# nnaisense/evotorch

Hardware: NVIDIA H100
Metric: PGPE generations/sec at popsize=1Mxdim=10k (Rastrigin, fp32) (higher is better)
Workload: dtype f32

## Files before the change

evotorch_b200/_native.py:

```python

from __future__ import annotations

import ctypes
import os
from ctypes import c_float, c_int, c_int64, c_size_t, c_uint64, c_void_p
from typing import Optional

import torch

_PKG = os.path.dirname(os.path.abspath(__file__))
LIB_PATH = os.path.join(_PKG, "lib", "libevok.so")

_P = c_void_p
_SIGNATURES = {
    "evok_abi_version": (c_int, []),
    "evok_launch_count": (c_uint64, []),
    "evok_error_string": (ctypes.c_char_p, [c_int]),
    "evok_sample_eval": (c_int, [c_int, _P, c_int64, _P, _P, c_int64, c_int64, c_int64, c_int, c_uint64, c_uint64, _P, _P, _P]),
    "evok_eval": (c_int, [c_int, _P, c_int64, c_int64, c_int64, _P, _P]),
    "evok_objective_register": (c_int, [_P, c_size_t, _P, c_int, _P]),
    "evok_objective_load": (c_int, [c_int]),
    "evok_rank_workspace_bytes": (c_size_t, [c_int64]),
    "evok_rank": (c_int, [c_int, _P, c_int64, c_int, _P, _P, _P, c_size_t, _P]),
    "evok_argsort": (c_int, [_P, c_int64, c_int, _P, _P, c_size_t, _P]),
    "evok_sample_batched": (c_int, [_P, c_int64, c_int64, _P, c_int64, _P, c_int64, c_int64, c_int64, c_int64, c_int, c_uint64, c_uint64, _P]),
    "evok_rank_batched": (c_int, [c_int, _P, c_int64, c_int64, c_int, _P, _P, c_size_t, _P]),
    "evok_elite_mask_batched": (c_int, [_P, c_int64, c_int64, c_int64, _P, _P, c_size_t, _P]),
    "evok_weights_adjust_batched": (c_int, [_P, c_int64, c_int64, c_int, _P]),
    "evok_grad_batched_workspace_bytes": (c_size_t, [c_int64, c_int64, c_int64]),
    "evok_grad_batched": (c_int, [c_int, _P, c_int64, c_int64, _P, _P, c_int64, _P, c_int64, c_int64, c_int64, c_int64, c_float, c_float, _P, _P, _P,
                                  c_size_t, _P]),
    "evok_clipup_batched": (c_int, [_P, c_int64, c_int64, _P, _P, _P, _P, _P, _P]),
    "evok_sigma_update_batched": (c_int, [_P, _P, c_int64, c_int64, _P, c_int, _P, _P, _P, _P]),
    "evok_rank_table": (c_int, [_P, c_int64, c_int, _P, _P, _P, c_size_t, _P]),
    "evok_cholesky_workspace_bytes": (c_size_t, [c_int64]),
    "evok_cholesky": (c_int, [_P, c_int64, c_int64, _P, c_int64, _P, c_size_t, _P]),
    "evok_cmaes_row_weights": (c_int, [_P, _P, c_int64, c_int64, c_int64, c_int, _P, _P, _P]),
    "evok_cmaes_vector_update": (c_int, [_P, _P, c_int64, _P, _P, _P, _P, _P, c_int64, _P, c_int, _P, _P, _P]),
    "evok_sample_eval_sq": (c_int, [c_int, _P, c_int64, _P, _P, c_int64, c_int64, c_int64, c_uint64, c_uint64, _P, _P, _P, _P]),
    "evok_sepcma_workspace_bytes": (c_size_t, [c_int64, c_int64]),
    "evok_sepcma_moments": (c_int, [_P, _P, c_int, c_int64, c_int64, c_int64, c_uint64, c_uint64, _P, _P, _P, _P, _P, c_size_t, _P]),
    "evok_sepcma_update": (c_int, [_P, _P, _P, c_int64, _P, _P, _P, _P, _P, _P, _P, _P, _P, _P, c_int64, _P, c_int, c_int64, c_float, c_float, _P,
                                   _P]),
    "evok_weights_adjust": (c_int, [_P, c_int64, c_int, _P]),
    "evok_elite_mask": (c_int, [_P, c_int64, c_int64, _P, _P, c_size_t, _P]),
    "evok_grad_workspace_bytes": (c_size_t, [c_int64, c_int64]),
    "evok_grad": (c_int, [c_int, _P, c_int64, _P, _P, _P, c_int64, c_int64, c_float, c_float, _P, _P, _P, c_size_t, _P]),
    "evok_grad_regen": (c_int, [c_int, _P, _P, _P, c_int64, c_int64, c_int64, c_uint64, c_uint64, _P, c_float, c_float, _P, _P, _P,
                                c_size_t, _P]),
    "evok_grad_hybrid": (c_int, [c_int, _P, c_int64, _P, _P, _P, c_int64, c_int64, c_int64, c_uint64, c_uint64, _P, c_int, c_float, c_float, _P,
                                 _P, _P, c_size_t, _P]),
    "evok_grad_auto_split": (c_int, [c_int64]),
    "evok_grad_power_limit_mw": (c_int64, [c_int]),
    "evok_clipup_step": (c_int, [_P, c_int64, _P, c_float, c_float, c_float, _P, _P, _P]),
    "evok_adam_step": (c_int, [_P, c_int64, _P, _P, c_int64, c_float, c_float, c_float, c_float, _P, _P, _P]),
    "evok_sgd_step": (c_int, [_P, c_int64, _P, c_int, c_float, c_float, _P, _P, _P]),
    "evok_axpy": (c_int, [_P, c_int64, c_float, _P, _P]),
    "evok_sigma_update": (c_int, [_P, _P, c_int64, c_float, c_int, _P, c_float, _P, c_float, _P, c_float, _P]),
    "evok_cem_finalize": (c_int, [_P, _P, _P, c_int64, c_int64, _P, _P, _P]),
    "evok_mlp_parameter_length": (c_int64, [c_int, _P]),
    "evok_mlp_forward": (c_int, [_P, c_int64, _P, c_int64, _P, c_int64, c_int64, c_int, _P, _P, _P]),
    "evok_mlp_forward_prep": (c_int, [_P, c_int64, _P, c_int64, _P, c_int64, c_int64, c_int, _P, _P, _P, _P, _P, c_float, c_float, c_float, _P, _P,
                                      c_size_t, _P]),
    "evok_mlp_forward_shared_supported": (c_int, [c_int, _P]),
    "evok_mlp_forward_shared_workspace_bytes": (c_size_t, [c_int64, c_int64, c_int, _P]),
    "evok_mlp_forward_shared": (c_int, [_P, c_int64, c_int64, _P, c_int64, c_int64, c_int, _P, _P, _P, _P, c_size_t, _P]),
    "evok_gemm_gather_rows": (c_int, [_P, c_int64, c_int64, c_int64, c_int64, _P, c_int64, c_int64, c_int64, c_int64, c_int, _P, c_int64, _P]),
    "evok_gemm_gather_rows_workspace_bytes": (c_size_t, [c_int64, c_int64]),
    "evok_gemm_gather_rows_ws": (c_int, [_P, c_int64, c_int64, c_int64, c_int64, _P, c_int64, c_int64, c_int64, c_int64, c_int, _P, c_int64, c_int, _P, c_size_t, _P]),
    "evok_gemm_workspace_bytes": (c_size_t, [c_int64, c_int64, c_int64]),
    "evok_gemm_nt": (c_int, [_P, c_int64, _P, c_int64, c_int64, c_int64, c_int64, _P, c_int64, _P, c_int64, _P, _P, _P, c_size_t, _P]),
    "evok_gemm_nt_affine": (c_int, [_P, c_int64, _P, c_int64, c_int64, c_int64, c_int64, _P, c_int64, _P, _P, c_int64, _P, _P, c_size_t, _P]),
    "evok_transpose_pair": (c_int, [_P, c_int64, c_int64, c_int64, _P, _P, _P, c_int64, _P]),
    "evok_transpose_scale": (c_int, [_P, c_int64, c_int64, c_int64, _P, _P, c_int64, _P]),
    "evok_peer_alloc": (c_int, [c_size_t, _P, _P]),
    "evok_peer_open": (c_int, [_P, _P]),
    "evok_peer_close": (c_int, [_P]),
    "evok_peer_free": (c_int, [_P]),
    "evok_sample_eval_push": (c_int, [c_int, _P, c_int64, _P, _P, c_int64, c_int64, c_int64, c_int, c_uint64, c_uint64, _P, c_int, c_int, _P, _P,
                                      _P, _P, _P]),
    "evok_peer_push": (c_int, [_P, c_int64, c_int64, c_int, c_int, _P, _P, _P, _P]),
    "evok_peer_wait": (c_int, [_P, c_int, _P, _P, c_uint64, _P]),
    "evok_grad_push": (c_int, [c_int, _P, c_int64, _P, _P, _P, c_int64, c_int64, c_int64, c_uint64, c_uint64, _P, c_float, c_float, c_int, c_int,
                               _P, _P, _P, _P, _P, c_size_t, _P]),
    "evok_rank_sharded": (c_int, [c_int, _P, c_int64, c_int, c_int, c_int, _P, _P, _P, _P, _P, _P, _P, c_uint64, _P, _P, _P, c_size_t, _P]),
    "evok_peer_reduce": (c_int, [_P, c_int, c_int64, _P, _P, _P, _P, c_uint64, _P, _P]),
}

EXPORTED_SYMBOLS = tuple(sorted(_SIGNATURES))

_lib: Optional[ctypes.CDLL] = None


class EvokError(RuntimeError):
    pass


def lib() -> ctypes.CDLL:
    global _lib
    if _lib is None:
        if not os.path.exists(LIB_PATH):
            raise EvokError(
                f"{LIB_PATH} is missing: the sm_90a kernel library has not been built. "
                "Run `python -m evotorch_b200.build` (needs nvcc). There is no CPU/torch fallback for CUDA problems."
# ... 72 lines not shown
```

evotorch_b200/csrc/evok_grad.cu:

```cuda
#include <dlfcn.h>

#include <atomic>
#include <cstdlib>

#include "evok_common.cuh"

#ifndef EVOK_GRAD_TMA_DEFAULT
#define EVOK_GRAD_TMA_DEFAULT 1
#endif

namespace evok {

#ifndef EVOK_GRAD_UNROLL
#define EVOK_GRAD_UNROLL 4
#endif
#ifndef EVOK_GRAD_MINB
#define EVOK_GRAD_MINB 4
#endif
#ifndef EVOK_GRAD_CTAS_PER_SM
#define EVOK_GRAD_CTAS_PER_SM 4
#endif
constexpr int kGradThreads = 256;
constexpr int kGradUnroll = EVOK_GRAD_UNROLL;
constexpr int kMaxResidentCtas = kNumSMs * 8;
// ... 199 lines not shown
  }
  out_mu[j] = t1 * scale_mu;
  out_sigma[j] = t2 * scale_sigma;
}

struct GradPush {
  PeerSink sink;
  const unsigned long long* epoch;
  unsigned int* done;
};

__global__ void __launch_bounds__(256) grad_finalize_push_kernel(const float* __restrict__ partial, int n_chunks, int64_t D, float scale_mu,
                                                                 float scale_sigma, const __grid_constant__ PeerSink sink,
                                                                 const unsigned long long* epoch, unsigned int* done) {
  const int64_t j = (int64_t)blockIdx.x * blockDim.x + threadIdx.x;
  if (j < D) {
    float t1 = 0.0f, t2 = 0.0f;
    for (int c = 0; c < n_chunks; ++c) {
      t1 += partial[((int64_t)c * 2 + 0) * D + j];
      t2 += partial[((int64_t)c * 2 + 1) * D + j];
    }
    t1 *= scale_mu;
    t2 *= scale_sigma;
    for (int p = 0; p < sink.world; ++p) {
      float* slot = static_cast<float*>(sink.data[p]) + (int64_t)sink.rank * 2 * D;
      slot[j] = t1;
      slot[D + j] = t2;
    }
  }
  peer_signal_tail(sink, epoch, done);
}

static int launch_finalize(const float* partial, int n_chunks, int64_t D, float scale_mu, float scale_sigma, float* out_mu, float* out_sigma,
                           const GradPush* push, cudaStream_t st) {
  const unsigned grid = (unsigned)((D + 255) / 256);
  if (push) grad_finalize_push_kernel<<<grid, 256, 0, st>>>(partial, n_chunks, D, scale_mu, scale_sigma, push->sink, push->epoch, push->done);
  else grad_finalize_kernel<<<grid, 256, 0, st>>>(partial, n_chunks, D, scale_mu, scale_sigma, out_mu, out_sigma);
  EVOK_CHECK_LAUNCH();
  return 0;
}

#ifndef EVOK_GRAD_TMA_ROWS
#define EVOK_GRAD_TMA_ROWS 4
#endif
#ifndef EVOK_GRAD_TMA_STAGES
#define EVOK_GRAD_TMA_STAGES 4
#endif
#ifndef EVOK_GRAD_TMA_CTAS_PER_SM
#define EVOK_GRAD_TMA_CTAS_PER_SM 3
#endif
constexpr int kTmaRows = EVOK_GRAD_TMA_ROWS;
constexpr int kTmaStages = EVOK_GRAD_TMA_STAGES;
constexpr int kTmaCols = 1024;
constexpr int kTmaConsumers = 256;
constexpr int kTmaThreads = kTmaConsumers + 32;
constexpr size_t kTmaSmemBytes = (size_t)kTmaStages * kTmaRows * kTmaCols * sizeof(float) + 2 * kTmaStages * sizeof(uint64_t) + 128;

__device__ __forceinline__ uint32_t smem_u32(const void* p) { return (uint32_t)__cvta_generic_to_shared(p); }
__device__ __forceinline__ void mbar_init(uint64_t* bar, uint32_t count) {
  asm volatile("mbarrier.init.shared::cta.b64 [%0], %1;" ::"r"(smem_u32(bar)), "r"(count) : "memory");
}
__device__ __forceinline__ void mbar_expect_tx(uint64_t* bar, uint32_t bytes) {
  asm volatile("mbarrier.arrive.expect_tx.shared::cta.b64 _, [%0], %1;" ::"r"(smem_u32(bar)), "r"(bytes) : "memory");
}
__device__ __forceinline__ void mbar_arrive(uint64_t* bar) {
  asm volatile("mbarrier.arrive.shared::cta.b64 _, [%0];" ::"r"(smem_u32(bar)) : "memory");
}
__device__ __forceinline__ void mbar_wait(uint64_t* bar, uint32_t parity) {
  asm volatile(
      "{\n"
      ".reg .pred P1;\n"
      "LAB_WAIT:\n"
      "mbarrier.try_wait.parity.shared::cta.b64 P1, [%0], %1;\n"
      "@P1 bra DONE;\n"
      "bra LAB_WAIT;\n"
      "DONE:\n"
      "}" ::"r"(smem_u32(bar)), "r"(parity) : "memory");
}
__device__ __forceinline__ void bulk_load(void* dst_smem, const void* src_gmem, uint32_t bytes, uint64_t* bar) {
  asm volatile("cp.async.bulk.shared::cluster.global.mbarrier::complete_tx::bytes [%0], [%1], %2, [%3];" ::"r"(smem_u32(dst_smem)),
               "l"(src_gmem), "r"(bytes), "r"(smem_u32(bar))
               : "memory");
}

constexpr int kSplitPeriod = 16;
__device__ __forceinline__ uint32_t rebuilt_mask(int split) {
  uint32_t m = 0;
#pragma unroll
  for (int k = 0; k < kSplitPeriod; ++k)
    if ((k + 1) * split / kSplitPeriod > k * split / kSplitPeriod) m |= 1u << k;
  return m;
}
__device__ __forceinline__ bool group_rebuilt(uint32_t mask, int64_t g) { return (mask >> ((int)g & (kSplitPeriod - 1))) & 1u; }

template <bool SYM>
__global__ void __launch_bounds__(kTmaThreads, EVOK_GRAD_TMA_CTAS_PER_SM)
    grad_partial_tma_kernel(int form, const float* __restrict__ X, int64_t ldx, const float* __restrict__ w, const float* __restrict__ mu,
                            const float* __restrict__ sigma, int64_t n_units, int64_t D, int64_t units_per_chunk, int split, uint64_t unit0,
                            const __grid_constant__ PhiloxKey key, const uint32_t* __restrict__ stream_off, float* __restrict__ partial) {
  extern __shared__ __align__(128) unsigned char smem_raw[];
  float* tiles = reinterpret_cast<float*>(smem_raw);
  uint64_t* full = reinterpret_cast<uint64_t*>(smem_raw + (size_t)kTmaStages * kTmaRows * kTmaCols * sizeof(float));
  uint64_t* empty = full + kTmaStages;

  const int tid = threadIdx.x, warp = tid >> 5, lane = tid & 31;
  const int64_t col0 = (int64_t)blockIdx.x * kTmaCols;
  const int64_t width = min((int64_t)kTmaCols, D - col0);
  const int64_t r_begin = (int64_t)blockIdx.y * units_per_chunk;
  const int64_t r_end = min(n_units, r_begin + units_per_chunk);
  const int64_t n_rows = r_end - r_begin;
  const int64_t n_groups = (n_rows + kTmaRows - 1) / kTmaRows;
  const int64_t row_stride = (SYM ? 2 : 1) * ldx;
  const uint32_t mask = rebuilt_mask(split);

  if (tid == 0) {
    for (int s = 0; s < kTmaStages; ++s) {
      mbar_init(&full[s], 1);
      mbar_init(&empty[s], kTmaConsumers / 32);
    }
    asm volatile("fence.mbarrier_init.release.cluster;" ::: "memory");
  }
  __syncthreads();

  if (warp == kTmaConsumers / 32) {
    if (lane == 0) {
      const uint32_t row_bytes = (uint32_t)(width * sizeof(float));
      int64_t t = 0;
      for (int64_t g = 0; g < n_groups; ++g) {
        if (group_rebuilt(mask, g)) continue;
        const int s = (int)(t % kTmaStages);
        const uint32_t use = (uint32_t)(t / kTmaStages);
        ++t;
        if (use > 0) mbar_wait(&empty[s], (use - 1) & 1);
        const int64_t r0 = r_begin + g * kTmaRows;
        const int rows = (int)min((int64_t)kTmaRows, r_end - r0);
        mbar_expect_tx(&full[s], rows * row_bytes);
        float* dst = tiles + (size_t)s * kTmaRows * kTmaCols;
        for (int i = 0; i < rows; ++i) bulk_load(dst + (size_t)i * kTmaCols, X + (r0 + i) * row_stride + col0, row_bytes, &full[s]);
      }
    }
    return;
  }

  const int64_t col = col0 + (int64_t)tid * 4;
  const bool active = col < D;
  const uint32_t sw = key.stream_lo + (stream_off ? __ldg(stream_off) : 0u);
  const int frm = SYM ? EVOK_GRAD_SYMMETRIC : form;
  float m[4], sg[4], c1[4], c0[4];
#pragma unroll
  for (int c = 0; c < 4; ++c) {
    sg[c] = active ? __ldg(sigma + col + c) : 1.0f;
    m[c] = active ? __ldg(mu + col + c) : 0.0f;
    if (frm == EVOK_GRAD_EXP) {
      c1[c] = __fdiv_rn(1.0f, sg[c] * sg[c]);
      c0[c] = 1.0f;
    } else if (frm == EVOK_GRAD_MOMENTS) {
      c1[c] = 1.0f;
      c0[c] = 0.0f;
    } else {
      c1[c] = __fdiv_rn(1.0f, sg[c]);
      c0[c] = sg[c];
    }
  }
  float s1[4] = {0.f, 0.f, 0.f, 0.f}, s2[4] = {0.f, 0.f, 0.f, 0.f};

  int64_t t = 0;
  for (int64_t g = 0; g < n_groups; ++g) {
    const int64_t r0 = r_begin + g * kTmaRows;
    const int rows = (int)min((int64_t)kTmaRows, r_end - r0);
    float a[kTmaRows], b[kTmaRows];
    bool need[kTmaRows];
#pragma unroll
    for (int i = 0; i < kTmaRows; ++i) {
      a[i] = b[i] = 0.0f;
      if (i < rows) {
        if (SYM) {
          const float wp = __ldg(w + 2 * (r0 + i)), wm = __ldg(w + 2 * (r0 + i) + 1);
          a[i] = 0.5f * (wp - wm);
          b[i] = 0.5f * (wp + wm);
        } else {
          a[i] = b[i] = __ldg(w + r0 + i);
        }
      }
      need[i] = a[i] != 0.0f || b[i] != 0.0f;
    }
    if (group_rebuilt(mask, g)) {
      if (active) {
        float x[kTmaRows][4];
#pragma unroll
        for (int i = 0; i < kTmaRows; ++i) {
          float z[4];
          normals4(key, sw, unit0 + (uint64_t)(r0 + i), (uint32_t)(col >> 2), z);
#pragma unroll
          for (int c = 0; c < 4; ++c) x[i][c] = fmaf(sg[c], z[c], m[c]);
        }
#pragma unroll
        for (int i = 0; i < kTmaRows; ++i) {
          if (need[i]) {
#pragma unroll
            for (int c = 0; c < 4; ++c) {
              const float e = x[i][c] - m[c];
              s1[c] = fmaf(a[i], e, s1[c]);
              s2[c] = fmaf(b[i], fmaf(e * e, c1[c], -c0[c]), s2[c]);
            }
          }
        }
      }
      continue;
    }
    const int s = (int)(t % kTmaStages);
    const uint32_t use = (uint32_t)(t / kTmaStages);
    ++t;
    mbar_wait(&full[s], use & 1);
    const float4* tile = reinterpret_cast<const float4*>(tiles + (size_t)s * kTmaRows * kTmaCols) + tid;
    if (active) {
      float4 v4[kTmaRows];
#pragma unroll
      for (int i = 0; i < kTmaRows; ++i) v4[i] = tile[(size_t)i * (kTmaCols / 4)];
#pragma unroll
      for (int i = 0; i < kTmaRows; ++i) {
        if (need[i]) {
          const float4 v = v4[i];
          const float x[4] = {v.x, v.y, v.z, v.w};
#pragma unroll
          for (int c = 0; c < 4; ++c) {
            const float e = x[c] - m[c];
            s1[c] = fmaf(a[i], e, s1[c]);
            s2[c] = fmaf(b[i], fmaf(e * e, c1[c], -c0[c]), s2[c]);
          }
        }
      }
    }
    __syncwarp();
    if (lane == 0) mbar_arrive(&empty[s]);
  }
  if (active) {
    float* p1 = partial + ((int64_t)blockIdx.y * 2 + 0) * D + col;
    float* p2 = partial + ((int64_t)blockIdx.y * 2 + 1) * D + col;
#pragma unroll
    for (int c = 0; c < 4; ++c) {
      p1[c] = s1[c];
      p2[c] = s2[c];
    }
  }
}

struct GradPlan {
  int vec, tx, n_coltiles, n_chunks;
  int64_t units_per_chunk;
};

static GradPlan plan_grad(int64_t n_units, int64_t D, bool vec_ok) {
  GradPlan p;
  p.vec = vec_ok ? 4 : 1;
  const int64_t col_threads = (D + p.vec - 1) / p.vec;
  p.tx = 32;
  while (p.tx < kGradThreads && p.tx < col_threads) p.tx <<= 1;
  p.n_coltiles = (int)((col_threads + p.tx - 1) / p.tx);
  const int ty = kGradThreads / p.tx;
  int64_t chunks = (int64_t)kNumSMs * EVOK_GRAD_CTAS_PER_SM / p.n_coltiles;
  const int64_t max_useful = (n_units + (int64_t)ty * kGradUnroll * 16 - 1) / ((int64_t)ty * kGradUnroll * 16);
  if (chunks > max_useful) chunks = max_useful;
  if (chunks < 1) chunks = 1;
  if (chunks > 65535) chunks = 65535;
  p.units_per_chunk = (n_units + chunks - 1) / chunks;
  p.n_chunks = (int)((n_units + p.units_per_chunk - 1) / p.units_per_chunk);
  if (p.n_chunks < 1) p.n_chunks = 1;
  return p;
}

template <int VEC, bool SYM, bool REGEN, bool SEPW = false>
static void launch_partial(const GradPlan& p, int form, const float* X, int64_t ldx, const float* w, const float* mu, const float* sigma,
                           int64_t n_units, int64_t D, uint64_t unit0, uint64_t seed, uint64_t stream_id, const uint32_t* stream_off, float* partial,
                           cudaStream_t st, int64_t n_items = 1, const GradItems* items = nullptr, const SepWeights* sep = nullptr) {
  dim3 grid(p.n_coltiles, p.n_chunks, (unsigned)n_items);
  const PhiloxKey key = make_philox_key(seed, stream_id);
  const GradItems it = items ? *items : GradItems{0, 0, 0, 0, 0};
  const SepWeights sw = sep ? *sep : SepWeights{nullptr, 0, nullptr};
#define EVOK_LAUNCH_TX(TXV)                                                                                                               \
  grad_partial_kernel<VEC, TXV, SYM, REGEN, SEPW><<<grid, kGradThreads, 0, st>>>(form, X, ldx, w, mu, sigma, n_units, D, p.units_per_chunk, \
                                                                                 unit0, key, stream_off, partial, it, sw)
  switch (p.tx) {
    case 32: EVOK_LAUNCH_TX(32); break;
    case 64: EVOK_LAUNCH_TX(64); break;
    case 128: EVOK_LAUNCH_TX(128); break;
    default: EVOK_LAUNCH_TX(256); break;
  }
#undef EVOK_LAUNCH_TX
}

constexpr int kAutoSplitCapped = 2;
constexpr int kAutoSplitFull = 5;
constexpr int64_t kFullPowerMilliwatts = 550000;

static int auto_split_for_power(int64_t milliwatts) { return milliwatts >= kFullPowerMilliwatts ? kAutoSplitFull : kAutoSplitCapped; }

static int64_t enforced_power_limit_mw(int device) {
  char bus_id[32];
  if (cudaDeviceGetPCIBusId(bus_id, (int)sizeof(bus_id), device) != cudaSuccess) {
    cudaGetLastError();
    return -1;
  }
  void* nvml = dlopen("libnvidia-ml.so.1", RTLD_NOW | RTLD_LOCAL);
  if (!nvml) return -1;
  using init_t = int (*)();
  using by_bus_t = int (*)(const char*, void**);
  using limit_t = int (*)(void*, unsigned int*);
  const auto init = reinterpret_cast<init_t>(dlsym(nvml, "nvmlInit_v2"));
  const auto shutdown = reinterpret_cast<init_t>(dlsym(nvml, "nvmlShutdown"));
  const auto by_bus = reinterpret_cast<by_bus_t>(dlsym(nvml, "nvmlDeviceGetHandleByPciBusId_v2"));
  const auto limit = reinterpret_cast<limit_t>(dlsym(nvml, "nvmlDeviceGetEnforcedPowerLimit"));
  int64_t mw = -1;
  if (init && shutdown && by_bus && limit && init() == 0) {
    void* handle = nullptr;
    unsigned int v = 0;
    if (by_bus(bus_id, &handle) == 0 && limit(handle, &v) == 0) mw = v;
    shutdown();
  }
  dlclose(nvml);
  return mw;
}

static int device_auto_split() {
  constexpr int kMaxDevices = 64;
  static std::atomic<int> resolved[kMaxDevices];
  int device = 0;
  if (cudaGetDevice(&device) != cudaSuccess || device < 0 || device >= kMaxDevices) {
    cudaGetLastError();
    return kAutoSplitCapped;
  }
  int s = resolved[device].load(std::memory_order_relaxed);
  if (s == 0) {
    s = auto_split_for_power(enforced_power_limit_mw(device)) + 1;
    resolved[device].store(s, std::memory_order_relaxed);
  }
  return s - 1;
}

static int grad_impl(int form, const float* X, int64_t ldx, const float* w, const float* mu, const float* sigma, int64_t row0, int64_t n_rows,
                     int64_t D, bool regen, uint64_t seed, uint64_t stream_id, const uint32_t* stream_off, float scale_mu, float scale_sigma, float* out_mu,
                     float* out_sigma, void* ws, size_t ws_bytes, void* stream, const GradPush* push = nullptr, int split = 0) {
  if ((!w && n_rows != 0) || !mu || !sigma || !ws || (!regen && !X) || (!push && (!out_mu || !out_sigma))) return EVOK_E_NULLPTR;
  if (form < EVOK_GRAD_SEPARABLE || form > EVOK_GRAD_MOMENTS) return EVOK_E_BADENUM;
  if (n_rows < 0 || D <= 0 || row0 < 0 || (!regen && ldx < D) || split < -1 || split > kSplitPeriod) return EVOK_E_BADSIZE;
  const bool sym = form == EVOK_GRAD_SYMMETRIC;
  if (sym && ((n_rows & 1) || (row0 & 1))) return EVOK_E_ODDROWS;
  if (ws_bytes < evok_grad_workspace_bytes(n_rows, D)) return EVOK_E_WORKSPACE;
  cudaStream_t st = (cudaStream_t)stream;
  const int64_t n_units = sym ? n_rows / 2 : n_rows;
  const bool vec_ok = regen ? true : ((D % 4 == 0) && (ldx % 4 == 0) && aligned16(X));
  const uint64_t unit0 = (uint64_t)(sym ? row0 / 2 : row0);
  float* partial = (float*)ws;
  if (n_units == 0 && push) return launch_finalize(partial, 0, D, scale_mu, scale_sigma, nullptr, nullptr, push, st);
  if (n_units == 0) {
    cudaMemsetAsync(out_mu, 0, (size_t)D * 4, st);
    cudaMemsetAsync(out_sigma, 0, (size_t)D * 4, st);
    return 0;
  }
  const GradPlan p = plan_grad(n_units, D, vec_ok);
  const char* tma_env = getenv("EVOK_GRAD_TMA");
  const int use_tma = tma_env ? atoi(tma_env) : EVOK_GRAD_TMA_DEFAULT;
  if (use_tma && !regen && vec_ok && form != EVOK_GRAD_MOMENTS && D >= 512 && n_units >= 4096) {
    const int n_coltiles = (int)((D + kTmaCols - 1) / kTmaCols);
    int64_t chunks = (int64_t)kNumSMs * EVOK_GRAD_TMA_CTAS_PER_SM / n_coltiles;
    if (chunks < 1) chunks = 1;
    if (chunks > 65535) chunks = 65535;
    const int64_t upc = (n_units + chunks - 1) / chunks;
    const int n_chunks = (int)((n_units + upc - 1) / upc);
    dim3 grid(n_coltiles, n_chunks);
    const int rebuilt = split < 0 ? device_auto_split() : split;
    const PhiloxKey key = make_philox_key(seed, stream_id);
    auto kernel = sym ? grad_partial_tma_kernel<true> : grad_partial_tma_kernel<false>;
    cudaFuncSetAttribute(kernel, cudaFuncAttributeMaxDynamicSharedMemorySize, (int)kTmaSmemBytes);
    kernel<<<grid, kTmaThreads, kTmaSmemBytes, st>>>(form, X, ldx, w, mu, sigma, n_units, D, upc, rebuilt, unit0, key, stream_off, partial);
    EVOK_CHECK_LAUNCH();
    return launch_finalize(partial, n_chunks, D, scale_mu, scale_sigma, out_mu, out_sigma, push, st);
  }
  if (regen) {
    if (sym) launch_partial<4, true, true>(p, form, X, ldx, w, mu, sigma, n_units, D, unit0, seed, stream_id, stream_off, partial, st);
    else launch_partial<4, false, true>(p, form, X, ldx, w, mu, sigma, n_units, D, unit0, seed, stream_id, stream_off, partial, st);
  } else if (vec_ok) {
    if (sym) launch_partial<4, true, false>(p, form, X, ldx, w, mu, sigma, n_units, D, unit0, seed, stream_id, stream_off, partial, st);
    else launch_partial<4, false, false>(p, form, X, ldx, w, mu, sigma, n_units, D, unit0, seed, stream_id, stream_off, partial, st);
  } else {
    if (sym) launch_partial<1, true, false>(p, form, X, ldx, w, mu, sigma, n_units, D, unit0, seed, stream_id, stream_off, partial, st);
    else launch_partial<1, false, false>(p, form, X, ldx, w, mu, sigma, n_units, D, unit0, seed, stream_id, stream_off, partial, st);
  }
  EVOK_CHECK_LAUNCH();
  return launch_finalize(partial, p.n_chunks, D, scale_mu, scale_sigma, out_mu, out_sigma, push, st);
}

}

using namespace evok;

extern "C" EVOK_API size_t evok_grad_workspace_bytes(int64_t n_rows, int64_t D) {
  (void)n_rows;
  if (D <= 0) return 256;
  return ((size_t)kMaxResidentCtas * 1024 + 2 * (size_t)D + 64) * sizeof(float);
}

extern "C" EVOK_API int evok_grad(int form, const float* X, int64_t ldx, const float* w, const float* mu, const float* sigma, int64_t n_rows,
                         int64_t D, float scale_mu, float scale_sigma, float* out_mu, float* out_sigma, void* ws, size_t ws_bytes,
                         void* stream) {
  return grad_impl(form, X, ldx, w, mu, sigma, 0, n_rows, D, false, 0, 0, nullptr, scale_mu, scale_sigma, out_mu, out_sigma, ws, ws_bytes, stream);
}

extern "C" EVOK_API int evok_grad_regen(int form, const float* w, const float* mu, const float* sigma, int64_t row0, int64_t n_rows, int64_t D,
                               uint64_t seed, uint64_t stream_id, const uint32_t* stream_offset_dev, float scale_mu, float scale_sigma,
                               float* out_mu, float* out_sigma, void* ws, size_t ws_bytes, void* stream) {
  return grad_impl(form, nullptr, 0, w, mu, sigma, row0, n_rows, D, true, seed, stream_id, stream_offset_dev, scale_mu, scale_sigma, out_mu, out_sigma, ws,
                   ws_bytes, stream);
}

extern "C" EVOK_API int evok_grad_hybrid(int form, const float* X, int64_t ldx, const float* w, const float* mu, const float* sigma, int64_t row0,
                                         int64_t n_rows, int64_t D, uint64_t seed, uint64_t stream_id, const uint32_t* stream_offset_dev, int split,
                                         float scale_mu, float scale_sigma, float* out_mu, float* out_sigma, void* ws, size_t ws_bytes, void* stream) {
  return grad_impl(form, X, ldx, w, mu, sigma, row0, n_rows, D, false, seed, stream_id, stream_offset_dev, scale_mu, scale_sigma, out_mu, out_sigma, ws,
                   ws_bytes, stream, nullptr, split);
}

extern "C" EVOK_API int evok_grad_auto_split(int64_t power_limit_mw) { return auto_split_for_power(power_limit_mw); }

extern "C" EVOK_API int64_t evok_grad_power_limit_mw(int device) { return enforced_power_limit_mw(device); }

extern "C" EVOK_API size_t evok_sepcma_workspace_bytes(int64_t n_rows, int64_t D) {
  return evok_grad_workspace_bytes(n_rows, D) + (size_t)kMaxResidentCtas * sizeof(float);
}

extern "C" EVOK_API int evok_sepcma_moments(const float* aw, const float* q, int active, int64_t row0, int64_t n_rows, int64_t D, uint64_t seed,
                                            uint64_t stream_id, const uint32_t* stream_offset_dev, float* local, float* S2, float* wsum, void* ws,
                                            size_t ws_bytes, void* stream) {
  if (!aw || (active && !q) || !local || !S2 || !wsum || !ws) return EVOK_E_NULLPTR;
  if (n_rows <= 0 || D <= 0 || row0 < 0) return EVOK_E_BADSIZE;
  if (ws_bytes < evok_sepcma_workspace_bytes(n_rows, D)) return EVOK_E_WORKSPACE;
  cudaStream_t st = (cudaStream_t)stream;
  const GradPlan p = plan_grad(n_rows, D, true);
  float* partial = (float*)ws;
  const SepWeights sep{q, active, partial + evok_grad_workspace_bytes(n_rows, D) / sizeof(float)};
  launch_partial<4, false, true, true>(p, EVOK_GRAD_MOMENTS, nullptr, 0, aw, nullptr, nullptr, n_rows, D, (uint64_t)row0, seed, stream_id,
                                       stream_offset_dev, partial, st, 1, nullptr, &sep);
  EVOK_CHECK_LAUNCH();
  grad_finalize_kernel<true><<<(unsigned)((D + 255) / 256), 256, 0, st>>>(partial, p.n_chunks, D, 1.0f, 1.0f, local, S2, 0, sep.wsum_partial, wsum);
  EVOK_CHECK_LAUNCH();
  return 0;
}

extern "C" EVOK_API int evok_grad_push(int form, const float* X, int64_t ldx, const float* w, const float* mu, const float* sigma, int64_t row0,
                                       int64_t n_rows, int64_t D, uint64_t seed, uint64_t stream_id, const uint32_t* stream_offset_dev,
                                       float scale_mu, float scale_sigma, int world, int rank, void* const* peer_slots, void* const* peer_flags,
                                       const uint64_t* epoch_dev, uint32_t* done_dev, void* ws, size_t ws_bytes, void* stream) {
  if (!peer_slots || !peer_flags || !epoch_dev || !done_dev) return EVOK_E_NULLPTR;
  if (world < 1 || world > EVOK_MAX_PEERS || rank < 0 || rank >= world) return EVOK_E_BADSIZE;
// ... 75 lines not shown
```

evotorch_b200/ops.py:

```python

from __future__ import annotations

import ctypes
import math
from typing import Optional

import torch

from . import _native as nat
from .tools.readonlytensor import as_plain_tensor

OBJ_NONE, OBJ_SPHERE, OBJ_RASTRIGIN, OBJ_ACKLEY = 0, 1, 2, 3
OBJ_USER_BASE = 64
OBJECTIVE_IDS = {"sphere": OBJ_SPHERE, "rastrigin": OBJ_RASTRIGIN, "ackley": OBJ_ACKLEY}
RANK_IDS = {"centered": 0, "linear": 1, "nes": 2, "normalized": 3, "raw": 4}
GRAD_SEPARABLE, GRAD_SYMMETRIC, GRAD_EXP, GRAD_MOMENTS = 0, 1, 2, 3
NAN = float("nan")


_timers: Optional[dict] = None


def enable_timers() -> None:
    global _timers
# ... 320 lines not shown
    nat.check(nat.lib().evok_elite_mask(w.data_ptr(), n, num_elites, mask.data_ptr(), ws.data_ptr(), ws.numel(), nat.stream_of(w)),
              "evok_elite_mask")
    return mask


def grad(form: int, X: torch.Tensor, w: torch.Tensor, mu: torch.Tensor, sigma: torch.Tensor, scale_mu: float, scale_sigma: float,
         out_mu: Optional[torch.Tensor] = None, out_sigma: Optional[torch.Tensor] = None) -> tuple:
    _mat(X, "samples")
    n, D = X.shape
    _vec(w, "weights", n); _vec(mu, "mu", D); _vec(sigma, "sigma", D)
    out_mu, out_sigma = _out_pair(mu, out_mu, out_sigma)
    ws = nat.workspace(X.device, nat.lib().evok_grad_workspace_bytes(n, D), "grad")
    with _timed("grad"):
        rc = nat.lib().evok_grad(form, X.data_ptr(), X.stride(0), w.data_ptr(), mu.data_ptr(), sigma.data_ptr(), n, D, scale_mu,
                                 scale_sigma, out_mu.data_ptr(), out_sigma.data_ptr(), ws.data_ptr(), ws.numel(), nat.stream_of(X))
    nat.check(rc, "evok_grad")
    return out_mu, out_sigma


def grad_regen(form: int, w: torch.Tensor, mu: torch.Tensor, sigma: torch.Tensor, *, seed: int, stream_id: int, row0: int,
               scale_mu: float, scale_sigma: float, out_mu: Optional[torch.Tensor] = None,
               out_sigma: Optional[torch.Tensor] = None, stream_offset: Optional[torch.Tensor] = None) -> tuple:
    n, D = w.numel(), mu.numel()
    _vec(w, "weights"); _vec(mu, "mu"); _vec(sigma, "sigma", D)
    out_mu, out_sigma = _out_pair(mu, out_mu, out_sigma)
    ws = nat.workspace(mu.device, nat.lib().evok_grad_workspace_bytes(n, D), "grad")
    with _timed("grad_regen"):
        rc = nat.lib().evok_grad_regen(form, w.data_ptr(), mu.data_ptr(), sigma.data_ptr(), row0, n, D, seed, stream_id,
                                       _offset_ptr(stream_offset), scale_mu, scale_sigma, out_mu.data_ptr(), out_sigma.data_ptr(),
                                       ws.data_ptr(), ws.numel(), nat.stream_of(mu))
    nat.check(rc, "evok_grad_regen")
    return out_mu, out_sigma


GRAD_SPLIT_PERIOD = 16


def grad_hybrid(form: int, X: torch.Tensor, w: torch.Tensor, mu: torch.Tensor, sigma: torch.Tensor, *, seed: int, stream_id: int, row0: int,
                scale_mu: float, scale_sigma: float, split: int = -1, out_mu: Optional[torch.Tensor] = None,
                out_sigma: Optional[torch.Tensor] = None, stream_offset: Optional[torch.Tensor] = None) -> tuple:
    _mat(X, "samples")
    n, D = X.shape
    _vec(w, "weights", n); _vec(mu, "mu", D); _vec(sigma, "sigma", D)
    if not -1 <= split <= GRAD_SPLIT_PERIOD:
        raise ValueError(f"split: expected -1 .. {GRAD_SPLIT_PERIOD}, got {split}")
    out_mu, out_sigma = _out_pair(mu, out_mu, out_sigma)
    ws = nat.workspace(X.device, nat.lib().evok_grad_workspace_bytes(n, D), "grad")
    with _timed("grad_hybrid"):
        rc = nat.lib().evok_grad_hybrid(form, X.data_ptr(), X.stride(0), w.data_ptr(), mu.data_ptr(), sigma.data_ptr(), row0, n, D,
                                        seed, stream_id, _offset_ptr(stream_offset), int(split), scale_mu, scale_sigma,
                                        out_mu.data_ptr(), out_sigma.data_ptr(), ws.data_ptr(), ws.numel(), nat.stream_of(X))
    nat.check(rc, "evok_grad_hybrid")
    return out_mu, out_sigma


def clipup_step(g: torch.Tensor, velocity: torch.Tensor, stepsize: float, momentum: float, max_speed: float,
                step_out: Optional[torch.Tensor] = None, mu: Optional[torch.Tensor] = None) -> None:
    D = g.numel()
    _vec(g, "g"); _vec(velocity, "velocity", D)
    with _timed("mu_step"):
        rc = nat.lib().evok_clipup_step(g.data_ptr(), D, velocity.data_ptr(), stepsize, momentum, max_speed, nat.ptr(step_out),
                                        nat.ptr(mu), nat.stream_of(g))
    nat.check(rc, "evok_clipup_step")


def adam_step(g: torch.Tensor, m: torch.Tensor, v: torch.Tensor, t: int, lr: float, beta1: float, beta2: float, eps: float,
              step_out: Optional[torch.Tensor] = None, mu: Optional[torch.Tensor] = None) -> None:
    D = g.numel()
    _vec(g, "g"); _vec(m, "m", D); _vec(v, "v", D)
    rc = nat.lib().evok_adam_step(g.data_ptr(), D, m.data_ptr(), v.data_ptr(), t, lr, beta1, beta2, eps, nat.ptr(step_out), nat.ptr(mu),
                                  nat.stream_of(g))
    nat.check(rc, "evok_adam_step")


def sgd_step(g: torch.Tensor, buf: Optional[torch.Tensor], first_step: bool, lr: float, momentum: float,
             step_out: Optional[torch.Tensor] = None, mu: Optional[torch.Tensor] = None) -> None:
    D = g.numel()
    _vec(g, "g")
    rc = nat.lib().evok_sgd_step(g.data_ptr(), D, nat.ptr(buf), int(first_step), lr, momentum, nat.ptr(step_out), nat.ptr(mu),
                                 nat.stream_of(g))
    nat.check(rc, "evok_sgd_step")


def axpy_(mu: torch.Tensor, g: torch.Tensor, lr: float) -> None:
    D = g.numel()
    _vec(g, "g"); _vec(mu, "mu", D)
    nat.check(nat.lib().evok_axpy(g.data_ptr(), D, lr, mu.data_ptr(), nat.stream_of(g)), "evok_axpy")


def _bound(x, D: int, device) -> tuple:
    if x is None:
        return None, NAN
    if isinstance(x, torch.Tensor) and x.ndim >= 1 and x.numel() > 1:
        v = x.to(device=device, dtype=torch.float32).contiguous()
        if v.numel() != D:
            raise IndexError(f"bound vector has length {v.numel()}, expected {D}")
        return v, NAN
    return None, float(x)


def sigma_update_(sigma: torch.Tensor, g: torch.Tensor, lr: float, exp_form: bool, lb=None, ub=None, max_change=None) -> None:
    D = sigma.numel()
    _vec(sigma, "sigma"); _vec(g, "g", D)
    lbv, lbs = _bound(lb, D, sigma.device)
    ubv, ubs = _bound(ub, D, sigma.device)
    mcv, mcs = _bound(max_change, D, sigma.device)
# ... 269 lines not shown
```

include/evok.h:

```cpp
#ifndef EVOK_H_
#define EVOK_H_

#ifndef __CUDACC_RTC__
#include <stddef.h>
#include <stdint.h>
#endif

#ifdef __cplusplus
extern "C" {
#endif

#define EVOK_ABI_VERSION 1

#if defined(__GNUC__)
#define EVOK_API __attribute__((visibility("default")))
#else
#define EVOK_API
#endif

#define EVOK_E_NULLPTR (-1)
#define EVOK_E_BADSIZE (-2)
#define EVOK_E_BADENUM (-3)
#define EVOK_E_WORKSPACE (-4)
#define EVOK_E_ODDROWS (-5)
// ... 15 lines not shown
#define EVOK_RANK_NES 2
#define EVOK_RANK_NORMALIZED 3
#define EVOK_RANK_RAW 4

#define EVOK_GRAD_SEPARABLE 0
#define EVOK_GRAD_SYMMETRIC 1
#define EVOK_GRAD_EXP 2
#define EVOK_GRAD_MOMENTS 3

int evok_abi_version(void);
uint64_t evok_launch_count(void);
const char* evok_error_string(int code);

int evok_sample_eval(int objective, float* X, int64_t ldx, const float* mu, const float* sigma, int64_t row0,
                     int64_t n_rows, int64_t D, int symmetric, uint64_t seed, uint64_t stream_id,
                     const uint32_t* stream_offset_dev, float* f, void* stream);

int evok_eval(int objective, const float* X, int64_t ldx, int64_t n_rows, int64_t D, float* f, void* stream);

#define EVOK_OBJ_KERNEL_SAMPLE 0
#define EVOK_OBJ_KERNEL_PUSH 8
#define EVOK_OBJ_KERNEL_SQ 16
#define EVOK_OBJ_KERNEL_EVAL 20
#define EVOK_OBJ_KERNELS 22
int evok_objective_register(const void* cubin, size_t bytes, const char* const* kernel_names_host, int n_kernels, int* id_out_host);
int evok_objective_load(int objective);

size_t evok_rank_workspace_bytes(int64_t N);
int evok_rank(int method, const float* f, int64_t N, int higher_is_better, float* w, int64_t* perm, void* ws,
              size_t ws_bytes, void* stream);

int evok_argsort(const float* keys, int64_t N, int descending, int64_t* perm, void* ws, size_t ws_bytes,
                 void* stream);

int evok_rank_table(const float* keys, int64_t N, int descending, const float* table, float* out, void* ws, size_t ws_bytes, void* stream);

int evok_weights_adjust(float* w, int64_t N, int mode, void* stream);

int evok_elite_mask(const float* w, int64_t N, int64_t num_elites, float* mask, void* ws, size_t ws_bytes,
                    void* stream);

size_t evok_grad_workspace_bytes(int64_t n_rows, int64_t D);
int evok_grad(int form, const float* X, int64_t ldx, const float* w, const float* mu, const float* sigma,
              int64_t n_rows, int64_t D, float scale_mu, float scale_sigma, float* out_mu, float* out_sigma,
              void* ws, size_t ws_bytes, void* stream);

int evok_grad_regen(int form, const float* w, const float* mu, const float* sigma, int64_t row0, int64_t n_rows,
                    int64_t D, uint64_t seed, uint64_t stream_id, const uint32_t* stream_offset_dev, float scale_mu,
                    float scale_sigma, float* out_mu, float* out_sigma, void* ws, size_t ws_bytes, void* stream);

int evok_grad_hybrid(int form, const float* X, int64_t ldx, const float* w, const float* mu, const float* sigma, int64_t row0,
                     int64_t n_rows, int64_t D, uint64_t seed, uint64_t stream_id, const uint32_t* stream_offset_dev, int split,
                     float scale_mu, float scale_sigma, float* out_mu, float* out_sigma, void* ws, size_t ws_bytes, void* stream);

int evok_grad_auto_split(int64_t power_limit_mw);

int64_t evok_grad_power_limit_mw(int device);

int evok_clipup_step(const float* g, int64_t D, float* velocity, float stepsize, float momentum, float max_speed,
                     float* step_out, float* mu, void* stream);
int evok_adam_step(const float* g, int64_t D, float* m, float* v, int64_t t, float lr, float beta1, float beta2,
                   float eps, float* step_out, float* mu, void* stream);
int evok_sgd_step(const float* g, int64_t D, float* buf, int first_step, float lr, float momentum, float* step_out,
                  float* mu, void* stream);
int evok_axpy(const float* g, int64_t D, float lr, float* mu, void* stream);

int evok_sigma_update(float* sigma, const float* g, int64_t D, float lr, int exp_form, const float* lb_vec,
                      float lb, const float* ub_vec, float ub, const float* mc_vec, float mc, void* stream);

int evok_cem_finalize(const float* s1, const float* s2, const float* sigma, int64_t D, int64_t num_elites,
                      float* grad_mu, float* grad_sigma, void* stream);

#define EVOK_ACT_NONE 0
#define EVOK_ACT_TANH 1
#define EVOK_ACT_RELU 2
#define EVOK_ACT_SIGMOID 3
int64_t evok_mlp_parameter_length(int n_layers, const int32_t* dims_host);
int evok_mlp_forward(const float* params, int64_t ldp, const float* obs, int64_t ldo, float* out, int64_t ldout, int64_t N,
                     int n_layers, const int32_t* dims_host, const int32_t* acts_host, void* stream);

int evok_mlp_forward_prep(const float* params, int64_t ldp, const float* obs, int64_t ldo, float* out, int64_t ldout, int64_t N,
                          int n_layers, const int32_t* dims_host, const int32_t* acts_host, const float* obs_sum, const float* obs_sumsq,
                          const int64_t* obs_count_dev, float min_variance, float clip_lo, float clip_hi, const uint8_t* active,
                          void* ws, size_t ws_bytes, void* stream);

int evok_mlp_forward_shared_supported(int n_layers, const int32_t* dims_host);
size_t evok_mlp_forward_shared_workspace_bytes(int64_t N, int64_t B, int n_layers, const int32_t* dims_host);
int evok_mlp_forward_shared(const float* params, int64_t ldp, int64_t N, const float* X, int64_t ldx, int64_t B, int n_layers,
                            const int32_t* dims_host, const int32_t* acts_host, float* out, void* ws, size_t ws_bytes, void* stream);
int evok_gemm_gather_rows(const float* params, int64_t batch_stride, int64_t w_offset, int64_t rows_per_batch, int64_t n_batches, const float* X,
                          int64_t ldx, int64_t n_cols, int64_t K, int64_t bias_offset, int act, float* C, int64_t ldc, void* stream);
size_t evok_gemm_gather_rows_workspace_bytes(int64_t n_cols, int64_t K);
int evok_gemm_gather_rows_ws(const float* params, int64_t batch_stride, int64_t w_offset, int64_t rows_per_batch, int64_t n_batches, const float* X,
                             int64_t ldx, int64_t n_cols, int64_t K, int64_t bias_offset, int act, float* C, int64_t ldc, int unit_fastest, void* ws,
                             size_t ws_bytes, void* stream);

size_t evok_gemm_workspace_bytes(int64_t M, int64_t N, int64_t K);
int evok_gemm_nt(const float* A, int64_t lda, const float* B, int64_t ldb, int64_t M, int64_t N, int64_t K, float* C, int64_t ldc,
                 float* C2, int64_t ldc2, const float* alpha_dev, const float* bias, void* ws, size_t ws_bytes, void* stream);
int evok_gemm_nt_affine(const float* A, int64_t lda, const float* B, int64_t ldb, int64_t M, int64_t N, int64_t K, float* C, int64_t ldc,
                        const float* k_dev, const float* E, int64_t lde, const float* u, void* ws, size_t ws_bytes, void* stream);
int evok_transpose_scale(const float* in, int64_t ldi, int64_t rows, int64_t cols, const float* w, float* out, int64_t ldo, void* stream);
int evok_transpose_pair(const float* in, int64_t ldi, int64_t rows, int64_t cols, const float* w, float* out_w, float* out_p, int64_t ldo,
                        void* stream);

int evok_sample_batched(float* X, int64_t item_stride_x, int64_t ldx, const float* mu, int64_t item_stride_mu, const float* sigma,
// ... 61 lines not shown
```

Before: 55.30.

## Split TMA grad kernel into warp-specialized loader and Philox rebuilder teams with dynamic claiming

Restructures the hybrid gradient kernel. A TMA producer warp and a separate team of 128 rebuilder threads both fill a shared smem ring. Rebuilders regenerate rows from Philox instead of reading X, and the consumers no longer compute normals inline. By default (split<0) each group is claimed dynamically through a shared atomic counter rather than a fixed static split, so the load/regenerate ratio adapts at runtime. Consumers drop to 128 threads, each handling two quads, and the kernel writes a per-CTA record of rebuilt groups so the host can read back the share. The trade-off is atomic contention, smem ring handoffs for rebuilt data, and higher register pressure in the consumers.

```diff
diff --git a/evotorch_b200/_native.py b/evotorch_b200/_native.py
--- a/evotorch_b200/_native.py
+++ b/evotorch_b200/_native.py
@@ -50,6 +50,7 @@
                                 c_size_t, _P]),
     "evok_grad_hybrid": (c_int, [c_int, _P, c_int64, _P, _P, _P, c_int64, c_int64, c_int64, c_uint64, c_uint64, _P, c_int, c_float, c_float, _P,
                                  _P, _P, c_size_t, _P]),
+    "evok_grad_schedule_offset": (c_size_t, [c_int64]),
     "evok_grad_auto_split": (c_int, [c_int64]),
     "evok_grad_power_limit_mw": (c_int64, [c_int]),
     "evok_clipup_step": (c_int, [_P, c_int64, _P, c_float, c_float, c_float, _P, _P, _P]),
diff --git a/evotorch_b200/csrc/evok_grad.cu b/evotorch_b200/csrc/evok_grad.cu
--- a/evotorch_b200/csrc/evok_grad.cu
+++ b/evotorch_b200/csrc/evok_grad.cu
@@ -275,9 +275,15 @@
 constexpr int kTmaRows = EVOK_GRAD_TMA_ROWS;
 constexpr int kTmaStages = EVOK_GRAD_TMA_STAGES;
 constexpr int kTmaCols = 1024;
-constexpr int kTmaConsumers = 256;
-constexpr int kTmaThreads = kTmaConsumers + 32;
-constexpr size_t kTmaSmemBytes = (size_t)kTmaStages * kTmaRows * kTmaCols * sizeof(float) + 2 * kTmaStages * sizeof(uint64_t) + 128;
+constexpr int kTmaConsumers = 128;
+constexpr int kTmaRebuilders = 128;
+constexpr int kTmaConsumerQuads = kTmaCols / 4 / kTmaConsumers;
+constexpr int kTmaRebuildQuads = kTmaCols / 4 / kTmaRebuilders;
+constexpr int kTmaProducerWarp = kTmaConsumers / 32;
+constexpr int kTmaRebuildWarp0 = kTmaProducerWarp + 1;
+constexpr int kTmaThreads = kTmaConsumers + 32 + kTmaRebuilders;
+constexpr size_t kTmaRingBytes = (size_t)kTmaStages * kTmaRows * kTmaCols * sizeof(float);
+constexpr size_t kTmaSmemBytes = kTmaRingBytes + 2 * kTmaStages * sizeof(uint64_t) + 128;
 
 __device__ __forceinline__ uint32_t smem_u32(const void* p) { return (uint32_t)__cvta_generic_to_shared(p); }
 __device__ __forceinline__ void mbar_init(uint64_t* bar, uint32_t count) {
@@ -306,6 +312,8 @@
                : "memory");
 }
 
+__device__ __forceinline__ void rebuilders_sync() { asm volatile("bar.sync 1, %0;" ::"n"(kTmaRebuilders) : "memory"); }
+
 constexpr int kSplitPeriod = 16;
 __device__ __forceinline__ uint32_t rebuilt_mask(int split) {
   uint32_t m = 0;
@@ -315,16 +323,31 @@
   return m;
 }
 __device__ __forceinline__ bool group_rebuilt(uint32_t mask, int64_t g) { return (mask >> ((int)g & (kSplitPeriod - 1))) & 1u; }
+
+__device__ __forceinline__ int64_t claim_group(unsigned int* next, int split, uint32_t mask, bool rebuild, int64_t prev, int64_t n_groups) {
+  if (split < 0) return (int64_t)atomicAdd(next, 1u);
+  int64_t g = prev + 1;
+  while (g < n_groups && group_rebuilt(mask, g) != rebuild) ++g;
+  if (g < n_groups) {
+    volatile unsigned int* turn = next;
+    while (*turn != (unsigned int)g) __nanosleep(32);
+    *turn = (unsigned int)g + 1u;
+  }
+  return g;
+}
 
 template <bool SYM>
 __global__ void __launch_bounds__(kTmaThreads, EVOK_GRAD_TMA_CTAS_PER_SM)
     grad_partial_tma_kernel(int form, const float* __restrict__ X, int64_t ldx, const float* __restrict__ w, const float* __restrict__ mu,
                             const float* __restrict__ sigma, int64_t n_units, int64_t D, int64_t units_per_chunk, int split, uint64_t unit0,
-                            const __grid_constant__ PhiloxKey key, const uint32_t* __restrict__ stream_off, float* __restrict__ partial) {
+                            const __grid_constant__ PhiloxKey key, const uint32_t* __restrict__ stream_off, float* __restrict__ partial,
+                            unsigned int* __restrict__ rebuilt) {
   extern __shared__ __align__(128) unsigned char smem_raw[];
   float* tiles = reinterpret_cast<float*>(smem_raw);
-  uint64_t* full = reinterpret_cast<uint64_t*>(smem_raw + (size_t)kTmaStages * kTmaRows * kTmaCols * sizeof(float));
+  uint64_t* full = reinterpret_cast<uint64_t*>(smem_raw + kTmaRingBytes);
   uint64_t* empty = full + kTmaStages;
+  unsigned int* next = reinterpret_cast<unsigned int*>(empty + kTmaStages);
+  unsigned int* team_group = next + 1;
 
   const int tid = threadIdx.x, warp = tid >> 5, lane = tid & 31;
   const int64_t col0 = (int64_t)blockIdx.x * kTmaCols;
@@ -334,26 +357,26 @@
   const int64_t n_rows = r_end - r_begin;
   const int64_t n_groups = (n_rows + kTmaRows - 1) / kTmaRows;
   const int64_t row_stride = (SYM ? 2 : 1) * ldx;
-  const uint32_t mask = rebuilt_mask(split);
+  const uint32_t mask = split < 0 ? 0u : rebuilt_mask(split);
 
   if (tid == 0) {
     for (int s = 0; s < kTmaStages; ++s) {
       mbar_init(&full[s], 1);
       mbar_init(&empty[s], kTmaConsumers / 32);
     }
+    *next = 0u;
     asm volatile("fence.mbarrier_init.release.cluster;" ::: "memory");
   }
   __syncthreads();
 
-  if (warp == kTmaConsumers / 32) {
+  if (warp == kTmaProducerWarp) {
     if (lane == 0) {
       const uint32_t row_bytes = (uint32_t)(width * sizeof(float));
-      int64_t t = 0;
-      for (int64_t g = 0; g < n_groups; ++g) {
-        if (group_rebuilt(mask, g)) continue;
-        const int s = (int)(t % kTmaStages);
-        const uint32_t use = (uint32_t)(t / kTmaStages);
-        ++t;
+      for (int64_t g = -1;;) {
+        g = claim_group(next, split, mask, false, g, n_groups);
+        if (g >= n_groups) break;
+        const int s = (int)(g % kTmaStages);
+        const uint32_t use = (uint32_t)(g / kTmaStages);
         if (use > 0) mbar_wait(&empty[s], (use - 1) & 1);
         const int64_t r0 = r_begin + g * kTmaRows;
         const int rows = (int)min((int64_t)kTmaRows, r_end - r0);
@@ -365,29 +388,98 @@
     return;
   }
 
-  const int64_t col = col0 + (int64_t)tid * 4;
-  const bool active = col < D;
-  const uint32_t sw = key.stream_lo + (stream_off ? __ldg(stream_off) : 0u);
+  if (warp >= kTmaRebuildWarp0) {
+    const int rt = tid - kTmaRebuildWarp0 * 32;
+    unsigned int filled = 0;
+    if (split != 0) {
+      const uint32_t sw = key.stream_lo + (stream_off ? __ldg(stream_off) : 0u);
+      float rm[kTmaRebuildQuads][4], rs[kTmaRebuildQuads][4];
+#pragma unroll
+      for (int k = 0; k < kTmaRebuildQuads; ++k) {
+        const int64_t col = col0 + 4 * (int64_t)(rt + k * kTmaRebuilders);
+#pragma unroll
+        for (int c = 0; c < 4; ++c) {
+          rs[k][c] = col < D ? __ldg(sigma + col + c) : 1.0f;
+          rm[k][c] = col < D ? __ldg(mu + col + c) : 0.0f;
+        }
+      }
+      for (int64_t g = -1;;) {
+        if (rt == 0) {
+          g = claim_group(next, split, mask, true, g, n_groups);
+          *team_group = (unsigned int)min(g, n_groups);
+        }
+        rebuilders_sync();
+        g = *team_group;
+        if (g >= n_groups) break;
+        const int s = (int)(g % kTmaStages);
+        const int64_t r0 = r_begin + g * kTmaRows;
+        float x[kTmaRebuildQuads][kTmaRows][4];
+#pragma unroll
+        for (int k = 0; k < kTmaRebuildQuads; ++k) {
+          const int q = rt + k * kTmaRebuilders;
+          if (4 * q < width) {
+#pragma unroll
+            for (int i = 0; i < kTmaRows; ++i) {
+              float z[4];
+              normals4(key, sw, unit0 + (uint64_t)(r0 + i), (uint32_t)((col0 >> 2) + q), z);
+#pragma unroll
+              for (int c = 0; c < 4; ++c) x[k][i][c] = fmaf(rs[k][c], z[c], rm[k][c]);
+            }
+          }
+        }
+        if (rt == 0 && g >= kTmaStages) mbar_wait(&empty[s], (uint32_t)(g / kTmaStages - 1) & 1);
+        rebuilders_sync();
+        float* slot = tiles + (size_t)s * kTmaRows * kTmaCols;
+#pragma unroll
+        for (int k = 0; k < kTmaRebuildQuads; ++k) {
+          const int q = rt + k * kTmaRebuilders;
+          if (4 * q < width) {
+#pragma unroll
+            for (int i = 0; i < kTmaRows; ++i)
+              reinterpret_cast<float4*>(slot + (size_t)i * kTmaCols)[q] = make_float4(x[k][i][0], x[k][i][1], x[k][i][2], x[k][i][3]);
+          }
+        }
+        asm volatile("fence.proxy.async.shared::cta;" ::: "memory");
+        rebuilders_sync();
+        if (rt == 0) mbar_arrive(&full[s]);
+        ++filled;
+      }
+    }
+    if (rt == 0) {
+      const unsigned int cell = blockIdx.y * gridDim.x + blockIdx.x;
+      if (cell == 0) rebuilt[0] = gridDim.x * gridDim.y;
+      rebuilt[1 + 2 * cell] = filled;
+      rebuilt[2 + 2 * cell] = (unsigned int)n_groups;
+    }
+    return;
+  }
+
+  int64_t col[kTmaConsumerQuads];
+  bool active[kTmaConsumerQuads];
   const int frm = SYM ? EVOK_GRAD_SYMMETRIC : form;
-  float m[4], sg[4], c1[4], c0[4];
-#pragma unroll
-  for (int c = 0; c < 4; ++c) {
-    sg[c] = active ? __ldg(sigma + col + c) : 1.0f;
-    m[c] = active ? __ldg(mu + col + c) : 0.0f;
-    if (frm == EVOK_GRAD_EXP) {
-      c1[c] = __fdiv_rn(1.0f, sg[c] * sg[c]);
-      c0[c] = 1.0f;
-    } else if (frm == EVOK_GRAD_MOMENTS) {
-      c1[c] = 1.0f;
-      c0[c] = 0.0f;
-    } else {
-      c1[c] = __fdiv_rn(1.0f, sg[c]);
-      c0[c] = sg[c];
-    }
-  }
-  float s1[4] = {0.f, 0.f, 0.f, 0.f}, s2[4] = {0.f, 0.f, 0.f, 0.f};
-
-  int64_t t = 0;
+  float m[kTmaConsumerQuads][4], c1[kTmaConsumerQuads][4], c0[kTmaConsumerQuads][4];
+#pragma unroll
+  for (int k = 0; k < kTmaConsumerQuads; ++k) {
+    col[k] = col0 + 4 * (int64_t)(tid + k * kTmaConsumers);
+    active[k] = col[k] < D;
+#pragma unroll
+    for (int c = 0; c < 4; ++c) {
+      const float sg = active[k] ? __ldg(sigma + col[k] + c) : 1.0f;
+      m[k][c] = active[k] ? __ldg(mu + col[k] + c) : 0.0f;
+      if (frm == EVOK_GRAD_EXP) {
+        c1[k][c] = __fdiv_rn(1.0f, sg * sg);
+        c0[k][c] = 1.0f;
+      } else if (frm == EVOK_GRAD_MOMENTS) {
+        c1[k][c] = 1.0f;
+        c0[k][c] = 0.0f;
+      } else {
+        c1[k][c] = __fdiv_rn(1.0f, sg);
+        c0[k][c] = sg;
+      }
+    }
+  }
+  float s1[kTmaConsumerQuads][4] = {}, s2[kTmaConsumerQuads][4] = {};
+
   for (int64_t g = 0; g < n_groups; ++g) {
     const int64_t r0 = r_begin + g * kTmaRows;
     const int rows = (int)min((int64_t)kTmaRows, r_end - r0);
@@ -407,63 +499,43 @@
       }
       need[i] = a[i] != 0.0f || b[i] != 0.0f;
     }
-    if (group_rebuilt(mask, g)) {
-      if (active) {
-        float x[kTmaRows][4];
-#pragma unroll
-        for (int i = 0; i < kTmaRows; ++i) {
-          float z[4];
-          normals4(key, sw, unit0 + (uint64_t)(r0 + i), (uint32_t)(col >> 2), z);
-#pragma unroll
-          for (int c = 0; c < 4; ++c) x[i][c] = fmaf(sg[c], z[c], m[c]);
-        }
+    const int s = (int)(g % kTmaStages);
+    mbar_wait(&full[s], (uint32_t)(g / kTmaStages) & 1);
+    const float4* tile = reinterpret_cast<const float4*>(tiles + (size_t)s * kTmaRows * kTmaCols) + tid;
+#pragma unroll
+    for (int k = 0; k < kTmaConsumerQuads; ++k) {
+      if (active[k]) {
+        float4 v4[kTmaRows];
+#pragma unroll
+        for (int i = 0; i < kTmaRows; ++i) v4[i] = tile[(size_t)i * (kTmaCols / 4) + k * kTmaConsumers];
 #pragma unroll
         for (int i = 0; i < kTmaRows; ++i) {
           if (need[i]) {
+            const float4 v = v4[i];
+            const float x[4] = {v.x, v.y, v.z, v.w};
 #pragma unroll
             for (int c = 0; c < 4; ++c) {
-              const float e = x[i][c] - m[c];
-              s1[c] = fmaf(a[i], e, s1[c]);
-              s2[c] = fmaf(b[i], fmaf(e * e, c1[c], -c0[c]), s2[c]);
+              const float e = x[c] - m[k][c];
+              s1[k][c] = fmaf(a[i], e, s1[k][c]);
+              s2[k][c] = fmaf(b[i], fmaf(e * e, c1[k][c], -c0[k][c]), s2[k][c]);
             }
           }
         }
       }
-      continue;
-    }
-    const int s = (int)(t % kTmaStages);
-    const uint32_t use = (uint32_t)(t / kTmaStages);
-    ++t;
-    mbar_wait(&full[s], use & 1);
-    const float4* tile = reinterpret_cast<const float4*>(tiles + (size_t)s * kTmaRows * kTmaCols) + tid;
-    if (active) {
-      float4 v4[kTmaRows];
-#pragma unroll
-      for (int i = 0; i < kTmaRows; ++i) v4[i] = tile[(size_t)i * (kTmaCols / 4)];
-#pragma unroll
-      for (int i = 0; i < kTmaRows; ++i) {
-        if (need[i]) {
-          const float4 v = v4[i];
-          const float x[4] = {v.x, v.y, v.z, v.w};
-#pragma unroll
-          for (int c = 0; c < 4; ++c) {
-            const float e = x[c] - m[c];
-            s1[c] = fmaf(a[i], e, s1[c]);
-            s2[c] = fmaf(b[i], fmaf(e * e, c1[c], -c0[c]), s2[c]);
-          }
-        }
-      }
     }
     __syncwarp();
     if (lane == 0) mbar_arrive(&empty[s]);
   }
-  if (active) {
-    float* p1 = partial + ((int64_t)blockIdx.y * 2 + 0) * D + col;
-    float* p2 = partial + ((int64_t)blockIdx.y * 2 + 1) * D + col;
-#pragma unroll
-    for (int c = 0; c < 4; ++c) {
-      p1[c] = s1[c];
-      p2[c] = s2[c];
+#pragma unroll
+  for (int k = 0; k < kTmaConsumerQuads; ++k) {
+    if (active[k]) {
+      float* p1 = partial + ((int64_t)blockIdx.y * 2 + 0) * D + col[k];
+      float* p2 = partial + ((int64_t)blockIdx.y * 2 + 1) * D + col[k];
+#pragma unroll
+      for (int c = 0; c < 4; ++c) {
+        p1[c] = s1[k][c];
+        p2[c] = s2[k][c];
+      }
     }
   }
 }
@@ -558,6 +630,10 @@
     resolved[device].store(s, std::memory_order_relaxed);
   }
   return s - 1;
+}
+
+static size_t grad_partial_bytes(int64_t D) {
+  return ((size_t)kMaxResidentCtas * 1024 + 2 * (size_t)D + 64) * sizeof(float);
 }
 
 static int grad_impl(int form, const float* X, int64_t ldx, const float* w, const float* mu, const float* sigma, int64_t row0, int64_t n_rows,
@@ -591,11 +667,17 @@
     const int64_t upc = (n_units + chunks - 1) / chunks;
     const int n_chunks = (int)((n_units + upc - 1) / upc);
     dim3 grid(n_coltiles, n_chunks);
-    const int rebuilt = split < 0 ? device_auto_split() : split;
+    int rebuilt = split;
+    if (split < 0) {
+      const char* claim_env = getenv("EVOK_GRAD_CLAIM");
+      if (claim_env && atoi(claim_env) == 0) rebuilt = device_auto_split();
+    }
     const PhiloxKey key = make_philox_key(seed, stream_id);
     auto kernel = sym ? grad_partial_tma_kernel<true> : grad_partial_tma_kernel<false>;
     cudaFuncSetAttribute(kernel, cudaFuncAttributeMaxDynamicSharedMemorySize, (int)kTmaSmemBytes);
-    kernel<<<grid, kTmaThreads, kTmaSmemBytes, st>>>(form, X, ldx, w, mu, sigma, n_units, D, upc, rebuilt, unit0, key, stream_off, partial);
+    unsigned int* record = reinterpret_cast<unsigned int*>(static_cast<char*>(ws) + grad_partial_bytes(D));
+    kernel<<<grid, kTmaThreads, kTmaSmemBytes, st>>>(form, X, ldx, w, mu, sigma, n_units, D, upc, rebuilt, unit0, key, stream_off, partial,
+                                                     record);
     EVOK_CHECK_LAUNCH();
     return launch_finalize(partial, n_chunks, D, scale_mu, scale_sigma, out_mu, out_sigma, push, st);
   }
@@ -620,8 +702,10 @@
 extern "C" EVOK_API size_t evok_grad_workspace_bytes(int64_t n_rows, int64_t D) {
   (void)n_rows;
   if (D <= 0) return 256;
-  return ((size_t)kMaxResidentCtas * 1024 + 2 * (size_t)D + 64) * sizeof(float);
-}
+  return grad_partial_bytes(D) + (1 + 2 * (size_t)kMaxResidentCtas) * sizeof(unsigned int);
+}
+
+extern "C" EVOK_API size_t evok_grad_schedule_offset(int64_t D) { return D <= 0 ? 0 : grad_partial_bytes(D); }
 
 extern "C" EVOK_API int evok_grad(int form, const float* X, int64_t ldx, const float* w, const float* mu, const float* sigma, int64_t n_rows,
                          int64_t D, float scale_mu, float scale_sigma, float* out_mu, float* out_sigma, void* ws, size_t ws_bytes,
diff --git a/evotorch_b200/ops.py b/evotorch_b200/ops.py
--- a/evotorch_b200/ops.py
+++ b/evotorch_b200/ops.py
@@ -396,6 +396,16 @@
                                         out_mu.data_ptr(), out_sigma.data_ptr(), ws.data_ptr(), ws.numel(), nat.stream_of(X))
     nat.check(rc, "evok_grad_hybrid")
     return out_mu, out_sigma
+
+
+def grad_rebuilt_share(X: torch.Tensor) -> float:
+    n, D = X.shape
+    lib = nat.lib()
+    ws = nat.workspace(X.device, lib.evok_grad_workspace_bytes(n, D), "grad")
+    off = lib.evok_grad_schedule_offset(D)
+    cells = int(ws[off:off + 4].view(torch.int32).item())
+    rec = ws[off + 4:off + 4 + 8 * cells].view(torch.int32).view(cells, 2).sum(0).tolist()
+    return rec[0] / rec[1] if rec[1] else 0.0
 
 
 def clipup_step(g: torch.Tensor, velocity: torch.Tensor, stepsize: float, momentum: float, max_speed: float,
diff --git a/include/evok.h b/include/evok.h
--- a/include/evok.h
+++ b/include/evok.h
@@ -91,6 +91,8 @@
 int evok_grad_hybrid(int form, const float* X, int64_t ldx, const float* w, const float* mu, const float* sigma, int64_t row0,
                      int64_t n_rows, int64_t D, uint64_t seed, uint64_t stream_id, const uint32_t* stream_offset_dev, int split,
                      float scale_mu, float scale_sigma, float* out_mu, float* out_sigma, void* ws, size_t ws_bytes, void* stream);
+
+size_t evok_grad_schedule_offset(int64_t D);
 
 int evok_grad_auto_split(int64_t power_limit_mw);
 
```

Result: faster. 57.06 (median of 6 runs) (+3.2%).
